# nidium/libapenetwork

Hardware: AMD Instinct MI355X
Metric: LZ4 GiB/s device-resident (compress+decompress), 1M×64KiB blocks, 1/2/4/8 GPU (higher is better)
Workload: dtype u8

## Files before the change

libapenetwork_amd/csrc/lz4_encode.hip:

```cpp
#include "lz4_gpu_internal.h"
#include <type_traits>

namespace apelz4 {

#ifdef APE_LZ4_STATS
__device__ unsigned long long g_enc_stats[16];
hipError_t enc_stats_read(unsigned long long *out, int reset) {
    hipError_t e = hipMemcpyFromSymbol(out, HIP_SYMBOL(g_enc_stats), sizeof(g_enc_stats));
    if (e == hipSuccess && reset) {
        unsigned long long z[16] = {0};
        e = hipMemcpyToSymbol(HIP_SYMBOL(g_enc_stats), z, sizeof(z));
    }
    return e;
}
#endif

namespace {

constexpr int kWavesPerEu = 7;

constexpr uint32_t kEagerLen = 12;
static_assert(kEagerLen + 4u == 16u, "in[T-4, T+kEagerLen) is one 16-byte load (loadv)");
constexpr uint32_t kEagerL = 12;
constexpr uint32_t kExt2 = 64;
constexpr uint32_t kGroups = 16;
constexpr uint32_t kRingE = 1024;
static_assert((kRingE & (kRingE - 1u)) == 0u && kRingE < 65536u,
              "the ring holds recent input, not the block's window (DESIGN.md 3.1.1)");
constexpr int kSmall = 128;
constexpr uint32_t kQ = 128;
constexpr uint32_t kFetchAt = 48, kEmitAll = 80, kChunkRecs = 64u / 4u;
static_assert((kQ & (kQ - 1u)) == 0u, "record ring indexed by & (kQ - 1)");
static_assert(kEmitAll - 1u + 2u * kChunkRecs <= kQ, "walker -> emitter record ring overflow");
static_assert(kFetchAt < kEmitAll, "a fetch precedes emit_all");
constexpr int kEmitEvery = 8;
constexpr uint32_t kStage = 512;
constexpr uint32_t kStageAlloc = kStage + 16u + 16u + 64u;


constexpr uint32_t I_TRUNC = 1u << 7, I_HASHABLE = 1u << 13;
static_assert(kEagerLen + kExt2 < 128u, "len fits 7 bits");

struct __attribute__((aligned(16))) EncLds {
    uint32_t ring[kRingE / 4 + 16];
    uint16_t tab[kHSize];
    uint2 info[64];
    uint2 q[kQ];
    uint32_t qn[2];
    uint8_t __attribute__((aligned(16))) stage[kStageAlloc];
};

template <int N>
__device__ __forceinline__ void vm_wait() {
    static_assert(N >= 0 && N < 16, "vmcnt");
    __builtin_amdgcn_s_waitcnt(N | (7 << 4) | (15 << 8));
}

__device__ __forceinline__ void shift_bytes(const uint32_t (&L)[8], int d, uint32_t (&X)[8]) {
    uint32_t T[8];
#pragma unroll
    for (int k = 0; k < 8; k++) T[k] = L[k];
    const bool down = d >= 0;
    const int ad = down ? d : -d, w = ad >> 2;
    const uint32_t r = (uint32_t)ad & 3u;
#pragma unroll
    for (int bit = 4; bit >= 1; bit >>= 1) {
        if (w & bit) {
            if (down) {
#pragma unroll
                for (int k = 0; k < 8; k++) T[k] = (k + bit < 8) ? T[k + bit] : 0u;
            } else {
#pragma unroll
                for (int k = 7; k >= 0; k--) T[k] = (k - bit >= 0) ? T[k - bit] : 0u;
            }
        }
    }
#pragma unroll
    for (int k = 0; k < 8; k++) {
        if (down) X[k] = __builtin_amdgcn_alignbyte(k + 1 < 8 ? T[k + 1] : 0u, T[k], r);
        else X[k] = r ? __builtin_amdgcn_alignbyte(T[k], k >= 1 ? T[k - 1] : 0u, 4u - r) : T[k];
    }
}

template <bool SMALL>
__device__ __forceinline__ void load32(gcu8 *in, int n, int pos, uint32_t (&X)[8],
                                       bool fast = false) {
    if (!SMALL && fast) {
        gcu8 *q = in + (uint32_t)pos;
        const uint4 a = gload16(q), b = gload16(q + 16);
        X[0] = a.x; X[1] = a.y; X[2] = a.z; X[3] = a.w;
        X[4] = b.x; X[5] = b.y; X[6] = b.z; X[7] = b.w;
        return;
    }
    if (SMALL) {
#pragma unroll
        for (int k = 0; k < 8; k++) X[k] = 0;
#pragma unroll
        for (int k = 0; k < 32; k++) {
            const int q = pos + k;
            if (q >= 0 && q < n) X[k >> 2] |= (uint32_t)in[(uint32_t)q] << (8 * (k & 3));
        }
        return;
    }
    const int ca = pos < 0 ? 0 : (pos > n - 32 ? n - 32 : pos);
    gcu8 *q = in + (uint32_t)ca;
    const uint4 a = gload16(q), b = gload16(q + 16);
    const uint32_t L[8] = {a.x, a.y, a.z, a.w, b.x, b.y, b.z, b.w};
    if (ca == pos) {
#pragma unroll
        for (int k = 0; k < 8; k++) X[k] = L[k];
    } else {
        const int d = pos - ca;
        shift_bytes(L, d < -31 ? -31 : (d > 31 ? 31 : d), X);
        if (d > 31 || d < -31) {
#pragma unroll
            for (int k = 0; k < 8; k++) X[k] = 0;
        }
    }
}

__device__ __forceinline__ uint32_t ffbl(uint32_t d) {
    uint32_t r;
    asm("v_ffbl_b32 %0, %1" : "=v"(r) : "v"(d));
    return r;
}
__device__ __forceinline__ uint32_t ffbh(uint32_t d) {
    uint32_t r;
    asm("v_ffbh_u32 %0, %1" : "=v"(r) : "v"(d));
    return r;
}

template <int K0, int NA, int NB>
__device__ __forceinline__ uint32_t first_diff_bit(const uint32_t (&A)[NA], const uint32_t (&B)[NB]) {
// ... 613 lines not shown
    E.pend = 0;
    const uint32_t s0 = E.o0 & 15u, end = s0 + E.tot;
    gu8 *out = B.dst + (E.o0 - s0);
    const uint32_t c0 = 16u * (uint32_t)lane;
    const uint64_t bigm = E.bigm;
    const uint32_t nfull = end >> 4;
    const bool head = E.part && s0 != 0u;
    if ((uint32_t)lane < umin(nfull, kStage / 16u + 1u) && !(head && lane == 0))
        gstore16(out + c0, *(const uint4 *)(S.stage + c0));
    if (head || (bigm && (end & 15u) && nfull <= kStage / 16u)) {
        const uint32_t pc = (head && lane == 0) ? 0u : 16u * nfull;
        const bool act = (head && lane == 0) || (bigm && (end & 15u) && lane == 1);
        const uint4 w = *(const uint4 *)(S.stage + (act ? pc : 0u));
        const uint32_t W[4] = {w.x, w.y, w.z, w.w};
#pragma unroll
        for (uint32_t t = 0; t < 16u; t++)
            if (act && pc + t >= s0 && pc + t < end) out[pc + t] = (uint8_t)(W[t >> 2] >> (8 * (t & 3)));
    }
    if (bigm) {
        vm_wait<0>();
        for (uint64_t m = bigm; m; m &= m - 1) {
            const int j = __builtin_ctzll(m);
            emit_one(B, lane, E.o0 - s0 + lane_val(E.r, j), lane_val(E.ba, j), lane_val(E.lit, j),
                     lane_val(E.mlm4, j), lane_val(E.off, j));
        }
        E.part = true;
    } else {
        if (lane == 0) {
            const uint4 t = *(const uint4 *)(S.stage + 16u * nfull);
            *(uint4 *)S.stage = t;
        }
        E.part = head && nfull == 0u;
    }
}

__device__ __forceinline__ void emit_step(EncLds &S, const Blk &B, int lane, Emit &E) {
    if (E.pend == 1) emit_lits(S, lane, E);
    else if (E.pend == 2) emit_heads(S, lane, E);
    else if (E.pend == 3) emit_copy(S, B, lane, E);
}
__device__ __forceinline__ void emit_all(EncLds &S, const Blk &B, int lane, Emit &E) {
    if (E.pend == 1) emit_lits(S, lane, E);
    if (E.pend == 2) emit_heads(S, lane, E);
    if (E.pend == 3) emit_copy(S, B, lane, E);
}

__device__ __forceinline__ void emit_tail(EncLds &S, const Blk &B, int lane, Emit &E) {
    const uint32_t s0 = E.o & 15u;
    if (!E.part && s0 != 0u && (uint32_t)lane < s0)
        B.dst[E.o - s0 + (uint32_t)lane] = S.stage[lane];
}

__device__ __forceinline__ void prefix_history(EncLds &S, const Blk &B, int lane) {
    const uint32_t D = 64u * (uint32_t)B.k0;
    constexpr int kU = 8;
    for (uint32_t v0 = 0; v0 < D; v0 += 192u * kU) {
        uint2 x[kU];
        bool ok[kU];
#pragma unroll
        for (int u = 0; u < kU; u++) {
            const uint32_t v = v0 + 192u * u + 3u * (uint32_t)lane;
            ok[u] = v < D && v + 8u <= B.un;
            x[u] = gload8(B.in + (ok[u] ? v : 0u));
        }
#pragma unroll
        for (int u = 0; u < kU; u++) {
            const uint32_t v = v0 + 192u * u + 3u * (uint32_t)lane;
            if (ok[u]) S.tab[hashk(x[u].x, x[u].y)] = (uint16_t)v;
        }
    }
    const uint32_t p = D - 64u + (uint32_t)lane;
    const uint8_t by = B.in[p];
    ((uint8_t *)S.ring)[p & (kRingE - 1)] = by;
    if (((D - 64u) & (kRingE - 1)) == 0u) ((uint8_t *)S.ring)[kRingE + lane] = by;
}

__device__ __forceinline__ void cdict_history(EncLds &S, const Blk &B, int lane) {
    const uint32_t p = B.D - 64u + (uint32_t)lane;
    const uint8_t by = B.win[p];
    ((uint8_t *)S.ring)[p & (kRingE - 1)] = by;
    if (((B.D - 64u) & (kRingE - 1)) == 0u) ((uint8_t *)S.ring)[kRingE + lane] = by;
}

template <bool SMALL, bool ACC, bool EXT = false>
__device__ __forceinline__ void encode_block(EncLds &S, const Blk &B, int wave, int lane,
                                             int *result, int *tail) {
    STATS_DECL
    const int k0 = B.k0;
    const int nch = B.nr >= (uint32_t)kMinLength ? B.nch : k0;
    const int nsteps = k0 + ((nch - k0 + 3) & ~1);

    if (wave == 1) {
        PSet P0, P1;
        auto pstep = [&](auto fast, int s, PSet &cur, PSet &nxt) {
            constexpr bool F = decltype(fast)::value;
            vm_wait<3>();
            STAT(9);
            prod_ring<F>(S, B, s + 2, lane, cur.X);
            uint32_t X6[6];
            prod_own(S, s + 1, lane, X6);
            prod_lookup<SMALL, F, EXT>(S, B, s + 2, lane, cur.X, cur.cT, cur.jL, cur.h, cur.Y);
            prod_load<SMALL, F, EXT>(B, s + 4, lane, cur.X);
            STAT(5);
            vm_wait<4>();
            STAT(9);
            prod_measure<SMALL, F, EXT>(S, B, s + 1, lane, X6, nxt.Y, nxt.cT, nxt.jL, nxt.h, nxt.q);
            STAT(5);
            __syncthreads();
            STAT(6);
            prod_stage2_issue<SMALL, F, EXT>(S, B, s + 1, lane, nxt.q, nxt.E);
            STAT(7);
            vm_wait<3>();
            STAT(9);
            prod_finish<SMALL, F, EXT>(S, B, s, lane, cur.q, cur.E);
            STAT(7);
            __syncthreads();
            STAT(8);
        };
        if constexpr (EXT) {
            if (k0 > 0) cdict_history(S, B, lane);
        } else {
            if (k0 > 0) prefix_history(S, B, lane);
        }
        if (nch > k0) {
            prod_load<SMALL, false, EXT>(B, k0, lane, P0.X);
            prod_load<SMALL, false, EXT>(B, k0 + 1, lane, P1.X);
            prod_ring(S, B, k0, lane, P0.X);
            prod_lookup<SMALL, false, EXT>(S, B, k0, lane, P0.X, P0.cT, P0.jL, P0.h, P0.Y);
            prod_load<SMALL, false, EXT>(B, k0 + 2, lane, P0.X);
            prod_ring(S, B, k0 + 1, lane, P1.X);
            prod_lookup<SMALL, false, EXT>(S, B, k0 + 1, lane, P1.X, P1.cT, P1.jL, P1.h, P1.Y);
            prod_load<SMALL, false, EXT>(B, k0 + 3, lane, P1.X);
            prod_ring(S, B, k0 + 2, lane, P0.X);
            uint32_t X6[6];
            prod_own(S, k0, lane, X6);
            prod_measure<SMALL, false, EXT>(S, B, k0, lane, X6, P0.Y, P0.cT, P0.jL, P0.h, P0.q);
            prod_stage2_issue<SMALL, false, EXT>(S, B, k0, lane, P0.q, P0.E);
        }
        __builtin_amdgcn_s_waitcnt(0);
        __syncthreads();
        constexpr int kFastEnd = 328;
        const int nfast_abs = SMALL ? 0 : (int)umin((uint32_t)(B.n >= kFastEnd ? (B.n - kFastEnd) / 64 + 1 : 0),
                                                    (uint32_t)nsteps);
        const int nfast = nfast_abs > k0 ? k0 + ((nfast_abs - k0) & ~1) : k0;
        int s = k0;
        for (; s < nfast; s += 2) {
            pstep(std::true_type{}, s, P0, P1);
            pstep(std::true_type{}, s + 1, P1, P0);
        }
        for (; s < nsteps; s += 2) {
            pstep(std::false_type{}, s, P0, P1);
            pstep(std::false_type{}, s + 1, P1, P0);
        }
        STATS_FLUSH_TID(g_enc_stats, 64);
        return;
    }
    if (wave == 0) {
        Walk W;
        uint32_t qn = 0;
        W.q = 64u * (uint32_t)k0;
        W.anchor = W.q;
        WalkOut O;
        __syncthreads();
        const int s2 = nch + 1;
        __syncthreads();
        __syncthreads();
        int s = k0 + 1;
        for (; s < s2; s++) {
            walk_chain<ACC, EXT>(S, B, s - 1, lane, W, O);
            STAT(0);
            __syncthreads();
            STAT(4);
            walk_finish<ACC>(B, s - 1, lane, W, O);
            walk_publish(S, B, s - 1, lane, O, qn);
            STAT_ADD(11, __popcll(O.members));
            STAT(1);
            STAT_ADD(10, 3);
            __syncthreads();
            STAT(3);
        }
        for (; s < nsteps; s++) {
            __syncthreads();
            __syncthreads();
        }
        STATS_FLUSH(g_enc_stats);
        return;
    }
    Emit E;
    E.o = 0;
    E.ein = 64u * (uint32_t)k0;
    E.qc = 0;
    E.last = k0;
    E.overflow = false;
    E.part = false;
    E.pend = 0;
    E.nv = false;
    E.o0 = E.tot = 0;
    E.bigm = 0;
    E.r = E.lit = E.mlm4 = E.off = E.ba = 0;
    __syncthreads();
    for (int s = k0; s < nsteps; s++) {
        const uint32_t qr = (uint32_t)__builtin_amdgcn_readfirstlane(S.qn[0]);
        const uint32_t avail = umax(qr, E.qc) - E.qc;
        if (E.pend == 0) {
            if (avail != 0u && (avail >= kFetchAt || s - E.last >= kEmitEvery)) {
                emit_fetch(S, B, lane, E, avail, s >= 12 ? 64u * (uint32_t)(s - 12) : 0u);
                E.last = s;
            }
        } else if (avail >= kEmitAll) {
            emit_all(S, B, lane, E);
        } else {
            emit_step(S, B, lane, E);
        }
        STAT(2);
        __syncthreads();
        STAT(14);
        if (E.pend == 1 || E.pend == 3) emit_step(S, B, lane, E);
        STAT(12);
        __syncthreads();
        STAT(15);
    }
    emit_all(S, B, lane, E);
    {
        const uint32_t rlo = B.nch > 16 ? 64u * (uint32_t)(B.nch - 16) : 0u;
        for (uint32_t left = (uint32_t)__builtin_amdgcn_readfirstlane(umax(S.qn[0], S.qn[1])) - E.qc; left;) {
            const uint32_t qc0 = E.qc;
            emit_fetch(S, B, lane, E, left, rlo);
            emit_all(S, B, lane, E);
            left -= E.qc - qc0;
        }
    }
    if (!E.overflow) emit_tail(S, B, lane, E);
    uint32_t last_run = 0;
    if (!E.overflow) {
        const uint32_t anchor = E.ein;
        const uint32_t lit = B.un - anchor;
        last_run = lit;
        const uint32_t hdr = 1u + ext_bytes(lit);
        const uint32_t total = E.o + hdr + lit;
        if (total > B.cap) {
            E.overflow = true;
        } else {
            if (lane == 0) {
                B.dst[E.o] = (uint8_t)((lit < 15u ? lit : 15u) << 4);
                put_len(B.dst + E.o + 1, lit);
            }
            wave_copy(B.in, B.dst, anchor, E.o + hdr, lit, lane);
            E.o = total;
        }
    }
    if (lane == 0) {
        *result = E.overflow ? 0 : (int)E.o;
        if (tail) *tail = E.overflow ? 0 : (int)last_run;
    }
    STAT_ADD(13, 1);
    STATS_FLUSH_TID(g_enc_stats, 128);
}

}

template <bool ACC>
__global__ void __launch_bounds__(192) __attribute__((amdgpu_waves_per_eu(kWavesPerEu)))
lz4_encode_kernel(BlockArgs a) {
    __shared__ EncLds S;
    const int b = blockIdx.x;
    const int tid = threadIdx.x;
    const int lane = tid & 63, wave = __builtin_amdgcn_readfirstlane(tid >> 6);

    Blk B;
    B.in = (gcu8 *)(a.src ? a.src[b] : a.src_base + (size_t)b * a.src_stride);
    B.dst = (gu8 *)(a.dst ? a.dst[b] : a.dst_base + (size_t)b * a.dst_stride);
    const int nr = a.src_size[b];
    const int icap = a.dst_cap ? a.dst_cap[b] : (int)a.dst_stride;
    if (nr < 0 || nr > kMaxBlock || icap < 0) {
        if (tid == 0) a.result[b] = (nr > kMaxBlock) ? kErange : 0;
        return;
    }
    int D = 0;
    if (a.dict_size) {
        const int pre = a.dict_size[b];
        D = (pre > 0 ? (pre < kMaxBlock - nr ? pre : kMaxBlock - nr) : 0) & ~63;
        if (D < 64) D = 0;
    }
    B.in -= D;
    B.n = D + nr;
    B.nr = (uint32_t)nr;
    B.k0 = D / 64;
    B.stride = ACC ? (a.accel < (1 << 20) ? (uint32_t)a.accel : 1u << 20) : 1u;
    B.cap = (uint32_t)icap;
    B.un = (uint32_t)B.n;
    B.mstart = B.un >= 12 ? B.un - 12 : 0;
    B.mlimit = B.un >= 5 ? B.un - 5 : 0;
    B.nch = (B.n + 63) / 64;

    for (int i = tid; i < kHSize / 8; i += 192) ((uint4 *)S.tab)[i] = make_uint4(0, 0, 0, 0);
    for (int i = tid; i < (int)(kRingE / 16 + 4); i += 192) ((uint4 *)S.ring)[i] = make_uint4(0, 0, 0, 0);
    if (tid == 0) S.qn[0] = S.qn[1] = 0u;
    __syncthreads();
    int *const tail = a.tail ? a.tail + b : nullptr;
    if (B.n < kSmall) encode_block<true, ACC>(S, B, wave, lane, &a.result[b], tail);
    else encode_block<false, ACC>(S, B, wave, lane, &a.result[b], tail);
}

__global__ void __launch_bounds__(192) __attribute__((amdgpu_waves_per_eu(kWavesPerEu)))
lz4_encode_cdict_kernel(BlockArgs a, const uint8_t *cd) {
    __shared__ EncLds S;
    const int b = blockIdx.x;
    const int tid = threadIdx.x;
    const int lane = tid & 63, wave = __builtin_amdgcn_readfirstlane(tid >> 6);

    const CDictHdr H = *(const CDictHdr *)cd;
#include "lz4_encode_cdict.inc"
}

__global__ void __launch_bounds__(192) __attribute__((amdgpu_waves_per_eu(kWavesPerEu)))
lz4_encode_cdicts_kernel(BlockArgs a, const uint8_t *const *cdicts) {
    __shared__ EncLds S;
    const int b = blockIdx.x;
    const int tid = threadIdx.x;
    const int lane = tid & 63, wave = __builtin_amdgcn_readfirstlane(tid >> 6);

    gcu8 *cd = (gcu8 *)message_object(cdicts, b);
    if (!cd) {
        if (tid == 0) a.result[b] = 0;
        return;
    }
    const CDictHdr H = object_header<true>(cd);
#include "lz4_encode_cdict.inc"
}

hipError_t launch_encode_cdicts(const BlockArgs &a, const void *const *cdicts, hipStream_t s) {
    if (a.nblocks <= 0) return hipSuccess;
    hipLaunchKernelGGL(lz4_encode_cdicts_kernel, dim3(a.nblocks), dim3(192), 0, s, a,
                       (const uint8_t *const *)cdicts);
    return hipGetLastError();
}

hipError_t launch_encode_cdict(const BlockArgs &a, const void *cdict, hipStream_t s) {
    if (a.nblocks <= 0) return hipSuccess;
    hipLaunchKernelGGL(lz4_encode_cdict_kernel, dim3(a.nblocks), dim3(192), 0, s, a,
                       (const uint8_t *)cdict);
    return hipGetLastError();
}

hipError_t launch_encode(const BlockArgs &a, hipStream_t s) {
    if (a.nblocks <= 0) return hipSuccess;
    if (a.accel > 1)
        hipLaunchKernelGGL(lz4_encode_kernel<true>, dim3(a.nblocks), dim3(192), 0, s, a);
    else
        hipLaunchKernelGGL(lz4_encode_kernel<false>, dim3(a.nblocks), dim3(192), 0, s, a);
    return hipGetLastError();
}

}
```

libapenetwork_amd/csrc/lz4_encode_cdict.inc:

```
    if (H.magic != kCdMagic || H.D > kCdMaxWin || (H.D & 63u) != 0u || H.max_src < 1u ||
        H.max_src > (uint32_t)kMaxBlock || H.D + H.max_src > (uint32_t)kMaxBlock) {
        if (tid == 0) a.result[b] = 0;
        return;
    }
    const int nr = a.src_size[b];
    const int icap = a.dst_cap[b];
    if (nr < 0 || nr > (int)H.max_src || icap < 0) {
        if (tid == 0) a.result[b] = (nr > (int)H.max_src) ? kErange : 0;
        return;
    }
    const int D = (int)H.D;
    Blk B;
    B.win = (gcu8 *)(cd + kCdWin + kCdFront);
    B.D = (uint32_t)D;
    B.in = (gcu8 *)a.src[b] - D;
    B.dst = (gu8 *)a.dst[b];
    B.n = D + nr;
    B.nr = (uint32_t)nr;
    B.k0 = D / 64;
    B.stride = 1u;
    B.cap = (uint32_t)icap;
    B.un = (uint32_t)B.n;
    B.mstart = B.un >= 12 ? B.un - 12 : 0;
    B.mlimit = B.un >= 5 ? B.un - 5 : 0;
    B.nch = (B.n + 63) / 64;

    const uint4 *img = (const uint4 *)(cd + kCdTab);
    for (int i = tid; i < kHSize / 8; i += 192) ((uint4 *)S.tab)[i] = img[i];
    for (int i = tid; i < (int)(kRingE / 16 + 4); i += 192) ((uint4 *)S.ring)[i] = make_uint4(0, 0, 0, 0);
    if (tid == 0) S.qn[0] = S.qn[1] = 0u;
    __syncthreads();
    if (B.n < kSmall) encode_block<true, false, true>(S, B, wave, lane, &a.result[b], nullptr);
    else encode_block<false, false, true>(S, B, wave, lane, &a.result[b], nullptr);
```

libapenetwork_amd/csrc/lz4_gpu_internal.h:

```cpp
#pragma once
#include <hip/hip_runtime.h>
#include <stdint.h>

namespace apelz4 {

constexpr int kMinMatch = 4;
constexpr int kLastLiterals = 5;
constexpr int kMFLimit = 12;
constexpr int kMinLength = 13;
constexpr int kMaxBlock = 65536;
constexpr int kErange = -2147483647 - 1;

typedef __attribute__((address_space(1))) const uint8_t gcu8;
typedef __attribute__((address_space(1))) uint8_t gu8;
typedef uint32_t u32x4_u __attribute__((ext_vector_type(4), aligned(1)));
typedef uint32_t u32x2_u __attribute__((ext_vector_type(2), aligned(1)));
typedef uint32_t u32_u __attribute__((aligned(1)));

__device__ __forceinline__ uint4 gload16(gcu8 *p) {
    const u32x4_u v = *(__attribute__((address_space(1))) const u32x4_u *)p;
    return make_uint4(v.x, v.y, v.z, v.w);
}
__device__ __forceinline__ uint2 gload8(gcu8 *p) {
    const u32x2_u v = *(__attribute__((address_space(1))) const u32x2_u *)p;
// ... 3 lines not shown
    return *(__attribute__((address_space(1))) const u32_u *)p;
}
__device__ __forceinline__ void gstore16(gu8 *p, uint4 v) {
    u32x4_u w;
    w.x = v.x; w.y = v.y; w.z = v.z; w.w = v.w;
    *(__attribute__((address_space(1))) u32x4_u *)p = w;
}
__device__ __forceinline__ void gstore4(gu8 *p, uint32_t v) {
    *(__attribute__((address_space(1))) u32_u *)p = v;
}

__device__ __forceinline__ int lane_id() { return (int)__lane_id(); }

__device__ __forceinline__ uint64_t wave_ballot(bool c) { return __builtin_amdgcn_ballot_w64(c); }
__device__ __forceinline__ bool wave_any(bool c) { return __builtin_amdgcn_ballot_w64(c) != 0; }
__device__ __forceinline__ bool lane_in(uint64_t m) { return __builtin_amdgcn_inverse_ballot_w64(m); }

template <int CTRL, int ROW_MASK = 0xF>
__device__ __forceinline__ uint32_t dpp(uint32_t old, uint32_t v) {
    return (uint32_t)__builtin_amdgcn_update_dpp((int)old, (int)v, CTRL, ROW_MASK, 0xF, false);
}
template <int CTRL>
__device__ __forceinline__ uint32_t dpp_z(uint32_t v) {
    return (uint32_t)__builtin_amdgcn_mov_dpp((int)v, CTRL, 0xF, 0xF, true);
}
constexpr int kDppRowShr1 = 0x111, kDppRowShr2 = 0x112, kDppRowShr4 = 0x114,
              kDppRowShr8 = 0x118, kDppBcast15 = 0x142, kDppBcast31 = 0x143,
              kDppWaveShr1 = 0x138, kDppWaveShl1 = 0x130;

__device__ __forceinline__ uint32_t wave_incl_sum(uint32_t x) {
    x += dpp<kDppRowShr1>(0u, x);
    x += dpp<kDppRowShr2>(0u, x);
    x += dpp<kDppRowShr4>(0u, x);
    x += dpp<kDppRowShr8>(0u, x);
    x += dpp<kDppBcast15, 0xA>(0u, x);
    x += dpp<kDppBcast31, 0xC>(0u, x);
    return x;
}

__device__ __forceinline__ uint32_t umax(uint32_t a, uint32_t b) { return a > b ? a : b; }
__device__ __forceinline__ uint32_t umin(uint32_t a, uint32_t b) { return a < b ? a : b; }

__device__ __forceinline__ uint32_t wave_incl_max(uint32_t x) {
    x = umax(x, dpp<kDppRowShr1>(0u, x));
    x = umax(x, dpp<kDppRowShr2>(0u, x));
    x = umax(x, dpp<kDppRowShr4>(0u, x));
    x = umax(x, dpp<kDppRowShr8>(0u, x));
    x = umax(x, dpp<kDppBcast15, 0xA>(0u, x));
    x = umax(x, dpp<kDppBcast31, 0xC>(0u, x));
    return x;
}

__device__ __forceinline__ uint32_t wave_shr1(uint32_t x, uint32_t first) {
    return dpp<kDppWaveShr1>(first, x);
}

__device__ __forceinline__ uint32_t wave_excl_scan(uint32_t v) {
    return wave_shr1(wave_incl_sum(v), 0u);
}

__device__ __forceinline__ uint32_t lane_val(uint32_t v, int l) {
    return (uint32_t)__builtin_amdgcn_readlane((int)v, l);
}

__device__ __forceinline__ uint32_t wave_first(uint32_t v) {
    return (uint32_t)__builtin_amdgcn_readfirstlane((int)v);
}
template <class T>
__device__ __forceinline__ T *wave_uniform(T *p) {
    const uint64_t v = (uint64_t)p;
    return (T *)((uint64_t)wave_first((uint32_t)(v >> 32)) << 32 | wave_first((uint32_t)v));
}

constexpr int kHSize = 7328;
static_assert(kHSize < 8192 && kHSize % 8 == 0, "table size");
constexpr int kKey = 7;

__device__ __forceinline__ uint32_t hashk(uint32_t x0, uint32_t x1) {
    static_assert(kKey == 7, "hashk covers bytes 0..6");
    const uint32_t hi = __builtin_amdgcn_alignbyte(x1, x0, 3u);
    const uint32_t v = (uint32_t)__umul24(x0, 0x9E3779u) + (uint32_t)__umul24(hi, 0xC2B2AEu) +
                       (uint32_t)__umul24((x1 >> 16) & 0xFFu, 0x27D4EBu);
    return __umulhi(v, (uint32_t)kHSize);
}

constexpr uint32_t kCdMagic = 0x44435A4Cu;
constexpr uint32_t kCdTab = 16u, kCdWin = kCdTab + 2u * (uint32_t)kHSize;
constexpr uint32_t kCdFront = 16u, kCdBack = 256u;
constexpr uint32_t kCdMaxWin = (uint32_t)kMaxBlock - 64u;
constexpr uint32_t kCdSize = kCdWin + kCdFront + (uint32_t)kMaxBlock + kCdBack;
static_assert(kCdWin % 16u == 0u && kCdSize % 16u == 0u, "prepared dictionary regions");
struct CDictHdr {
    uint32_t magic, D, max_src, zero;
};
__device__ __forceinline__ const uint8_t *message_object(const uint8_t *const *objs, int b) {
    const uint8_t *cd = wave_uniform(objs[b]);
    return ((uint64_t)cd & 15u) ? nullptr : cd;
}
template <bool PER, class P>
__device__ __forceinline__ CDictHdr object_header(P *cd) {
    if constexpr (!PER) {
        return *(const CDictHdr *)cd;
    } else {
        const uint4 v = gload16((gcu8 *)cd);
        return CDictHdr{wave_first(v.x), wave_first(v.y), wave_first(v.z), wave_first(v.w)};
    }
}
__host__ __device__ inline int cdict_window(int dict_size, int max_src) {
    const int room = kMaxBlock - max_src;
    return (dict_size < room ? dict_size : room) & ~63;
}

#ifdef APE_LZ4_STATS
#define STATS_DECL uint64_t st_t_ = clock64(); uint64_t st_acc_[16] = {0};
#define STAT(i) do { uint64_t t_ = clock64(); st_acc_[i] += t_ - st_t_; st_t_ = t_; } while (0)
#define STAT_ADD(i, v) (st_acc_[i] += (uint64_t)(v))
#define STATS_FLUSH(arr) STATS_FLUSH_TID(arr, 0)
#define STATS_FLUSH_TID(arr, t) do { if (threadIdx.x == (t)) { _Pragma("unroll") for (int i_ = 0; i_ < 16; i_++) if (st_acc_[i_]) atomicAdd(&(arr)[i_], (unsigned long long)st_acc_[i_]); } } while (0)
#else
#define STATS_DECL
#define STAT(i) do {} while (0)
#define STAT_ADD(i, v) do {} while (0)
#define STATS_FLUSH(arr) do {} while (0)
#define STATS_FLUSH_TID(arr, t) do {} while (0)
#endif
hipError_t stats_read(int which, unsigned long long *out, int reset);

struct BlockArgs {
    const char *const *src;
    char *const *dst;
    const char *src_base;
    char *dst_base;
    size_t src_stride, dst_stride;
    const int *src_size;
    const int *dst_cap;
    const int *target;
    const long long *frame_off;
    const char *const *dict;
    const int *dict_size;
    int fast;
    int accel;
    int *result;
    int nblocks;
    int *tail;
};

hipError_t launch_decode(const BlockArgs &a, bool partial, hipStream_t s);
hipError_t launch_decode_chain(const BlockArgs &a, int nconn, int nq, hipStream_t s);
hipError_t launch_encode(const BlockArgs &a, hipStream_t s);
hipError_t launch_encode_cdict(const BlockArgs &a, const void *cdict, hipStream_t s);
hipError_t launch_encode_cdicts(const BlockArgs &a, const void *const *cdicts, hipStream_t s);
hipError_t launch_cdict_prepare(const char *dict, int dict_size, int max_src, void *cdict,
                                hipStream_t s);
hipError_t launch_cdict_prepare_batch(const char *const *dict, const int *dict_size, int max_src,
                                      void *cdicts, size_t stride, int n, hipStream_t s);
hipError_t launch_encode_exact(const BlockArgs &a, hipStream_t s);
constexpr int kHcCap = 272;
constexpr int kHcHashBits = 14;
constexpr int kHcMaxDepth = 256, kHcDefaultDepth = 64;
constexpr int kHcTable = 1 << kHcHashBits;
__device__ __forceinline__ uint32_t hc_hash(uint32_t x) {
    return (x * 2654435761u) >> (32 - kHcHashBits);
}
__device__ __forceinline__ uint32_t len_bytes(uint32_t v) { return v >= 15u ? (v - 15u) / 255u + 1u : 0u; }
__device__ __forceinline__ uint32_t first_diff(uint32_t x) { return (uint32_t)__builtin_ctz(x) >> 3; }
constexpr size_t kHcChainBytes = (size_t)kMaxBlock * sizeof(uint16_t);
constexpr size_t kHcSlotBytes = kHcChainBytes + (size_t)kMaxBlock * sizeof(uint32_t);
struct HcArgs {
    const char *const *src;
    const int *src_size;
    char *const *dst;
    const int *dst_cap;
    int *result;
    int nblocks, depth;
    uint16_t *chain;
    uint32_t *match;
    const int *prefix;
    int *tail;
};
hipError_t launch_encode_hc(const HcArgs &a, hipStream_t s, hipEvent_t *ev = nullptr);
constexpr size_t kHcOptSlotBytes = kHcSlotBytes + (size_t)kMaxBlock * sizeof(uint32_t);
struct HcOptArgs {
    HcArgs a;
    uint32_t *cost;
};
hipError_t launch_encode_hc_opt(const HcOptArgs &o, hipStream_t s, hipEvent_t *ev = nullptr);

constexpr uint32_t kHdMagic = 0x44485A4Cu;
constexpr uint32_t kHdHead = 16u, kHdChain = kHdHead + 2u * (1u << kHcHashBits);
constexpr uint32_t kHdWin = kHdChain + 2u * (uint32_t)kMaxBlock;
constexpr uint32_t kHdSize = kHdWin + kCdFront + (uint32_t)kMaxBlock + kCdBack;
static_assert(kHdChain % 16u == 0u && kHdWin % 16u == 0u && kHdSize % 16u == 0u,
              "prepared high-ratio dictionary regions");
__host__ __device__ inline int hc_cdict_window(int dict_size, int max_src) {
    const int room = kMaxBlock - max_src;
    return dict_size < room ? dict_size : room;
}
inline size_t hc_cdict_chain_entries(int max_src) { return ((size_t)max_src + 3 + 7) & ~(size_t)7; }
inline size_t hc_cdict_match_entries(int max_src) { return ((size_t)max_src + 3) & ~(size_t)3; }
inline size_t hc_cdict_slot_bytes(int max_src) {
    return hc_cdict_chain_entries(max_src) * sizeof(uint16_t) +
           hc_cdict_match_entries(max_src) * sizeof(uint32_t);
}
constexpr int kHcdThreads = 256;
inline int hc_cdict_groups(int max_src) { return (max_src + kHcdThreads - 1) / kHcdThreads; }
struct HcDictArgs {
    const char *const *src;
    const int *src_size;
    char *const *dst;
    const int *dst_cap;
    int *result;
    int nblocks, depth;
    int max_src;
    const uint8_t *cdict;
    uint16_t *chain;
    uint32_t *match;
    uint32_t chain_stride, match_stride;
};
hipError_t launch_hc_cdict_prepare(const char *dict, int dict_size, int max_src, void *cdict,
                                   hipStream_t s);
hipError_t launch_hc_cdict_prepare_batch(const char *const *dict, const int *dict_size,
                                         int max_src, void *cdicts, size_t stride, int n,
                                         hipStream_t s);
hipError_t launch_encode_hc_cdict(const HcDictArgs &a, hipStream_t s,
                                  const uint8_t *const *cdicts = nullptr);
inline size_t hc_cdict_cost_entries(int max_src) { return ((size_t)max_src + 3) & ~(size_t)3; }
inline size_t hc_cdict_opt_slot_bytes(int max_src) {
    return hc_cdict_slot_bytes(max_src) + hc_cdict_cost_entries(max_src) * sizeof(uint32_t);
}
struct HcDictOptArgs {
    HcDictArgs a;
    uint32_t *cost;
// ... 123 lines not shown
```

libapenetwork_amd/csrc/lz4_runtime.hip:

```cpp
#include <initializer_list>
#include <mutex>
#include <stdarg.h>
#include <stdio.h>
#include <string.h>
#include <vector>

#include "../../include/ape_lz4_gpu.h"
#include "lz4_gpu_internal.h"
#include "lz4_gpu_shim.h"

using namespace apelz4;

namespace {

thread_local char g_err[256] = "";

void set_err(const char *what, hipError_t e) {
    snprintf(g_err, sizeof g_err, "%s: %s", what, e == hipSuccess ? "ok" : hipGetErrorString(e));
}

__attribute__((format(printf, 1, 2))) int einval(const char *fmt, ...) {
    va_list ap;
    va_start(ap, fmt);
    vsnprintf(g_err, sizeof g_err, fmt, ap);
// ... 1104 lines not shown
    if (int rc = ready_strided("compress_batch_strided_dev", a)) return rc;
    return finish_launch(launch_encode(a, (hipStream_t)stream), "lz4_encode_kernel");
}

int APE_LZ4_decompress_safe_batch_strided_dev(const char *d_src, size_t src_stride,
                                              const int *d_compressedSize, char *d_dst,
                                              size_t dst_stride, const int *d_maxDecompressedSize,
                                              int *d_result, int nblocks, void *stream) {
    BlockArgs a = strided_args(d_src, src_stride, d_compressedSize, d_dst, dst_stride,
                               d_maxDecompressedSize, d_result, nblocks);
    if (int rc = ready_strided("decompress_safe_batch_strided_dev", a)) return rc;
    return finish_launch(launch_decode(a, false, (hipStream_t)stream), "lz4_decode_kernel");
}

size_t APE_LZ4_frame_scratch_size(int nblocks) {
    return nblocks < 0 ? 0 : (size_t)frame_scratch_elems(nblocks) * sizeof(long long);
}

int APE_LZ4_frame_offsets_dev(const int *d_compressedSize, long long *d_off,
                              void *d_scratch, int nblocks, void *stream) {
    if (nblocks < 0 || !d_compressedSize || !d_off || !d_scratch)
        return einval("frame_offsets_dev: invalid argument (a null array or a negative count, "
                      "nblocks %d)", nblocks);
    if (int rc = check_device()) return rc;
    return finish_launch(launch_frame_offsets(d_compressedSize, d_off, (long long *)d_scratch,
                                              nblocks, (hipStream_t)stream),
                         "frame offsets");
}

int APE_LZ4_frame_pack_strided_dev(const char *d_comp, size_t comp_stride,
                                   const int *d_compressedSize, const long long *d_off,
                                   char *d_frames, int nblocks, void *stream) {
    if (int rc = check_arrays("frame_pack_strided_dev", nblocks,
                              {d_comp, d_compressedSize, d_off, d_frames}))
        return rc;
    if (int rc = check_device()) return rc;
    return finish_launch(launch_frame_pack(d_comp, comp_stride, d_compressedSize, d_off,
                                           d_frames, nblocks, (hipStream_t)stream),
                         "frame pack");
}

int APE_LZ4_decompress_safe_frames_dev(const char *d_frames, const long long *d_off,
                                       char *d_dst, size_t dst_stride,
                                       const int *d_maxDecompressedSize, int *d_result,
                                       int nblocks, void *stream) {
    BlockArgs a = strided_args(d_frames, 0, nullptr, d_dst, dst_stride, d_maxDecompressedSize,
                               d_result, nblocks);
    a.frame_off = d_off;
    if (int rc = ready_strided("decompress_safe_frames_dev", a)) return rc;
    return finish_launch(launch_decode(a, false, (hipStream_t)stream), "lz4_decode_kernel");
}

int APE_LZ4_compress_batch_host(const char *const *h_src, const int *h_srcSize,
                                char *const *h_dst, const int *h_dstCap, int *h_result,
                                int nblocks) {
    return host_batch("compress_batch_host", 0, 1, h_src, h_srcSize, h_dst, h_dstCap, nullptr,
                      h_result, nblocks);
}

int APE_LZ4_decompress_safe_batch_host(const char *const *h_src, const int *h_compressedSize,
                                       char *const *h_dst, const int *h_maxDecompressedSize,
                                       int *h_result, int nblocks) {
    return host_batch("decompress_safe_batch_host", 1, 1, h_src, h_compressedSize, h_dst,
                      h_maxDecompressedSize, nullptr, h_result, nblocks);
}

int APE_LZ4_synth_blocks_dev(char *d_out, size_t stride, int blockSize, long long first_block,
                             int nblocks, int kind, void *stream) {
    if (nblocks < 0 || blockSize < 0 || blockSize > kMaxBlock || (nblocks > 0 && !d_out) ||
        stride < (size_t)blockSize)
        return einval("synth_blocks_dev: nblocks %d of %d bytes (0..%d) at %p with stride %zu",
                      nblocks, blockSize, kMaxBlock, d_out, stride);
    if (int rc = check_device()) return rc;
    return finish_launch(launch_synth(d_out, stride, blockSize, first_block, nblocks, kind,
                                      (hipStream_t)stream),
                         "lz4_synth_kernel");
}

#ifdef APE_LZ4_STATS
}
namespace apelz4 {
hipError_t dec_stats_read(unsigned long long *out, int reset);
hipError_t enc_stats_read(unsigned long long *out, int reset);
}
extern "C" {
int APE_LZ4_debug_stats(int which, unsigned long long *out16, int reset) {
    hipError_t e = which ? apelz4::enc_stats_read(out16, reset) : apelz4::dec_stats_read(out16, reset);
    return e == hipSuccess ? 0 : -1;
}
#endif

int ape_lz4_gpu_compress_one(const char *src, char *dst, int n, int cap, int accel, int *rt) {
    int res = 0;
    *rt = host_batch("compress_one", 0, accel, &src, &n, &dst, &cap, nullptr, &res, 1);
    return res;
}

int ape_lz4_gpu_decompress_one(const char *src, char *dst, int csize, int cap, int partial,
                               int target, int *rt) {
    int res = 0;
    *rt = host_batch("decompress_one", partial ? 2 : 1, 1, &src, &csize, &dst, &cap,
                     partial ? &target : nullptr, &res, 1);
    return res;
}

}
```

Before: 148.0.

## Assign encoder wave roles dynamically by per-SIMD load across CUs

Each encode workgroup reads its hardware CU and SIMD IDs and consults a global per-SIMD load table. It then permutes the walker, producer and emitter roles so the heavy producer wave lands on the least-loaded SIMD, and releases the load weight when it finishes. This targets imbalance when several resident blocks put their producer waves on the same SIMD. In exchange it adds global atomics per block, an extra barrier, and getreg reads, and it only runs for blocks of at least 32 KiB in auto mode.

```diff
diff --git a/libapenetwork_amd/csrc/lz4_encode.hip b/libapenetwork_amd/csrc/lz4_encode.hip
--- a/libapenetwork_amd/csrc/lz4_encode.hip
+++ b/libapenetwork_amd/csrc/lz4_encode.hip
@@ -10,6 +10,40 @@
     if (e == hipSuccess && reset) {
         unsigned long long z[16] = {0};
         e = hipMemcpyToSymbol(HIP_SYMBOL(g_enc_stats), z, sizeof(z));
+    }
+    return e;
+}
+#endif
+
+__device__ int g_enc_load[kEncCus * 4];
+static int g_role_mode = kEncRoleAuto;
+int enc_role_mode_set(int mode) {
+    if (mode < 0 || mode > kEncNPerms) return -1;
+    const int old = g_role_mode;
+    g_role_mode = mode;
+    return old;
+}
+hipError_t enc_loads_read(int *out) {
+    return hipMemcpyFromSymbol(out, HIP_SYMBOL(g_enc_load), sizeof(g_enc_load));
+}
+#ifdef APE_LZ4_STATS
+__device__ unsigned long long g_enc_place[64];
+__device__ int g_enc_prod[kEncCus * 4];
+__device__ int g_enc_seen[kEncCus];
+hipError_t enc_place_read(unsigned long long *out, int reset) {
+    unsigned long long h[64];
+    static int seen[kEncCus];
+    hipError_t e = hipMemcpyFromSymbol(h, HIP_SYMBOL(g_enc_place), sizeof(h));
+    if (e == hipSuccess) e = hipMemcpyFromSymbol(seen, HIP_SYMBOL(g_enc_seen), sizeof(seen));
+    if (e != hipSuccess) return e;
+    h[53] = 0;
+    for (int i = 0; i < kEncCus; i++) h[53] += seen[i] != 0;
+    for (int i = 0; i < 64; i++) out[i] = h[i];
+    if (reset) {
+        for (int i = 0; i < 64; i++) h[i] = 0;
+        for (int i = 0; i < kEncCus; i++) seen[i] = 0;
+        e = hipMemcpyToSymbol(HIP_SYMBOL(g_enc_place), h, sizeof(h));
+        if (e == hipSuccess) e = hipMemcpyToSymbol(HIP_SYMBOL(g_enc_seen), seen, sizeof(seen));
     }
     return e;
 }
@@ -47,8 +81,12 @@
     uint2 info[64];
     uint2 q[kQ];
     uint32_t qn[2];
+    uint8_t simd[4];
+    uint32_t perm;
     uint8_t __attribute__((aligned(16))) stage[kStageAlloc];
 };
+
+static_assert(sizeof(EncLds) <= 35 * 512, "35 LDS granules of 512 bytes: 9 blocks per CU");
 
 template <int N>
 __device__ __forceinline__ void vm_wait() {
@@ -828,15 +866,83 @@
     if (((B.D - 64u) & (kRingE - 1)) == 0u) ((uint8_t *)S.ring)[kRingE + lane] = by;
 }
 
+__device__ __forceinline__ uint32_t hw_simd() {
+    return __builtin_amdgcn_s_getreg(4 | 4 << 6 | (2 - 1) << 11);
+}
+__device__ __forceinline__ uint32_t hw_cu() {
+    const uint32_t cu = __builtin_amdgcn_s_getreg(4 | 8 << 6 | (8 - 1) << 11);
+    const uint32_t xcc = __builtin_amdgcn_s_getreg(20 | 0 << 6 | (4 - 1) << 11);
+    return (xcc << 8 | cu) & (uint32_t)(kEncCus - 1);
+}
+
+[[maybe_unused]] constexpr int kEncPlaceMin = 32768;
+__device__ __forceinline__ bool place_wanted(int mode, int nr) {
+#ifdef APE_LZ4_STATS
+    return true;
+#else
+    return mode == kEncRoleAuto && nr >= kEncPlaceMin;
+#endif
+}
+__device__ __forceinline__ int fixed_role(int mode, int wave) {
+    return enc_role(mode == kEncRoleAuto ? 0 : (int)umin((uint32_t)mode - 1u, kEncNPerms - 1u), wave);
+}
+
+__device__ __forceinline__ int place_begin(EncLds &S, int tid, int wave) {
+    if ((tid & 63) == 0) S.simd[wave] = (uint8_t)hw_simd();
+    int ld = 0;
+    if (tid < 4) ld = __hip_atomic_load(&g_enc_load[hw_cu() * 4u + (uint32_t)tid], __ATOMIC_RELAXED,
+                                        __HIP_MEMORY_SCOPE_AGENT);
+    return ld;
+}
+__device__ __forceinline__ int place_roles(EncLds &S, int mode, int ld, int tid, int wave) {
+    if (wave == 0) {
+        const int load[4] = {(int)lane_val((uint32_t)ld, 0), (int)lane_val((uint32_t)ld, 1),
+                             (int)lane_val((uint32_t)ld, 2), (int)lane_val((uint32_t)ld, 3)};
+        if (tid == 0) {
+            const int sd[3] = {S.simd[0] & 3, S.simd[1] & 3, S.simd[2] & 3};
+            const int k = mode != kEncRoleAuto ? mode - 1 : enc_place_roles(sd, load);
+            const uint32_t cu = hw_cu();
+#pragma unroll
+            for (int w = 0; w < kEncRoles; w++)
+                atomicAdd(&g_enc_load[cu * 4u + (uint32_t)sd[w]], enc_weight(enc_role(k, w)));
+            uint32_t post = (uint32_t)k | cu << 16;
+#ifdef APE_LZ4_STATS
+            {
+                int pw = 0;
+                for (int w = 0; w < kEncRoles; w++) if (enc_role(k, w) == 1) pw = w;
+                const int c = atomicAdd(&g_enc_prod[cu * 4u + (uint32_t)sd[pw]], 1);
+                post |= (uint32_t)(c < 0 ? 0 : c > 15 ? 15 : c) << 8;
+                g_enc_seen[cu] = 1;
+                if (sd[0] == sd[1] || sd[0] == sd[2] || sd[1] == sd[2]) atomicAdd(&g_enc_place[48], 1ull);
+                atomicAdd(&g_enc_place[49], 1ull);
+                atomicMax(&g_enc_place[50], (unsigned long long)umax(umax(S.simd[0], S.simd[1]), S.simd[2]));
+                atomicMax(&g_enc_place[51], (unsigned long long)__builtin_amdgcn_s_getreg(20 | (4 - 1) << 11));
+                atomicOr(&g_enc_place[52], (unsigned long long)__builtin_amdgcn_s_getreg(4 | 8 << 6 | (8 - 1) << 11));
+            }
+#endif
+            S.perm = post;
+        }
+    }
+    __syncthreads();
+    const int k = (int)umin(wave_first(S.perm) & 7u, (uint32_t)kEncNPerms - 1u);
+    return enc_role(k, wave);
+}
+__device__ __forceinline__ uint32_t place_entry(const EncLds &S, int wave) {
+    return (wave_first(S.perm) >> 16 & (uint32_t)(kEncCus - 1)) * 4u + (wave_first(S.simd[wave]) & 3u);
+}
+__device__ __forceinline__ void place_release(const EncLds &S, int wave, int role, int lane) {
+    if (lane == 0) atomicSub(&g_enc_load[place_entry(S, wave)], enc_weight(role));
+}
+
 template <bool SMALL, bool ACC, bool EXT = false>
-__device__ __forceinline__ void encode_block(EncLds &S, const Blk &B, int wave, int lane,
+__device__ __forceinline__ void encode_block(EncLds &S, const Blk &B, int role, int lane,
                                              int *result, int *tail) {
     STATS_DECL
     const int k0 = B.k0;
     const int nch = B.nr >= (uint32_t)kMinLength ? B.nch : k0;
     const int nsteps = k0 + ((nch - k0 + 3) & ~1);
 
-    if (wave == 1) {
+    if (role == 1) {
         PSet P0, P1;
         auto pstep = [&](auto fast, int s, PSet &cur, PSet &nxt) {
             constexpr bool F = decltype(fast)::value;
@@ -890,6 +996,9 @@
                                                     (uint32_t)nsteps);
         const int nfast = nfast_abs > k0 ? k0 + ((nfast_abs - k0) & ~1) : k0;
         int s = k0;
+#ifdef APE_LZ4_STATS
+        const uint64_t place_t0 = clock64();
+#endif
         for (; s < nfast; s += 2) {
             pstep(std::true_type{}, s, P0, P1);
             pstep(std::true_type{}, s + 1, P1, P0);
@@ -898,10 +1007,19 @@
             pstep(std::false_type{}, s, P0, P1);
             pstep(std::false_type{}, s + 1, P1, P0);
         }
-        STATS_FLUSH_TID(g_enc_stats, 64);
+#ifdef APE_LZ4_STATS
+        if (lane == 0 && nsteps > k0) {
+            const uint32_t c = wave_first(S.perm) >> 8 & 15u;
+            atomicAdd(&g_enc_place[c], 1ull);
+            atomicAdd(&g_enc_place[16 + c], (unsigned long long)(clock64() - place_t0));
+            atomicAdd(&g_enc_place[32 + c], (unsigned long long)(nsteps - k0));
+        }
+        if (lane == 0) atomicSub(&g_enc_prod[place_entry(S, (int)(threadIdx.x >> 6))], 1);
+#endif
+        STATS_FLUSH_TID(g_enc_stats, threadIdx.x & ~63u);
         return;
     }
-    if (wave == 0) {
+    if (role == 0) {
         Walk W;
         uint32_t qn = 0;
         W.q = 64u * (uint32_t)k0;
@@ -929,7 +1047,7 @@
             __syncthreads();
             __syncthreads();
         }
-        STATS_FLUSH(g_enc_stats);
+        STATS_FLUSH_TID(g_enc_stats, threadIdx.x & ~63u);
         return;
     }
     Emit E;
@@ -1000,7 +1118,7 @@
         if (tail) *tail = E.overflow ? 0 : (int)last_run;
     }
     STAT_ADD(13, 1);
-    STATS_FLUSH_TID(g_enc_stats, 128);
+    STATS_FLUSH_TID(g_enc_stats, threadIdx.x & ~63u);
 }
 
 }
@@ -1039,13 +1157,17 @@
     B.mlimit = B.un >= 5 ? B.un - 5 : 0;
     B.nch = (B.n + 63) / 64;
 
+    const bool placed = place_wanted(a.role_mode, nr);
+    const int ld = placed ? place_begin(S, tid, wave) : 0;
     for (int i = tid; i < kHSize / 8; i += 192) ((uint4 *)S.tab)[i] = make_uint4(0, 0, 0, 0);
     for (int i = tid; i < (int)(kRingE / 16 + 4); i += 192) ((uint4 *)S.ring)[i] = make_uint4(0, 0, 0, 0);
     if (tid == 0) S.qn[0] = S.qn[1] = 0u;
     __syncthreads();
+    const int role = placed ? place_roles(S, a.role_mode, ld, tid, wave) : fixed_role(a.role_mode, wave);
     int *const tail = a.tail ? a.tail + b : nullptr;
-    if (B.n < kSmall) encode_block<true, ACC>(S, B, wave, lane, &a.result[b], tail);
-    else encode_block<false, ACC>(S, B, wave, lane, &a.result[b], tail);
+    if (B.n < kSmall) encode_block<true, ACC>(S, B, role, lane, &a.result[b], tail);
+    else encode_block<false, ACC>(S, B, role, lane, &a.result[b], tail);
+    if (placed) place_release(S, wave, role, lane);
 }
 
 __global__ void __launch_bounds__(192) __attribute__((amdgpu_waves_per_eu(kWavesPerEu)))
@@ -1075,22 +1197,31 @@
 #include "lz4_encode_cdict.inc"
 }
 
-hipError_t launch_encode_cdicts(const BlockArgs &a, const void *const *cdicts, hipStream_t s) {
-    if (a.nblocks <= 0) return hipSuccess;
+static BlockArgs with_role_mode(const BlockArgs &a) {
+    BlockArgs b = a;
+    b.role_mode = g_role_mode;
+    return b;
+}
+
+hipError_t launch_encode_cdicts(const BlockArgs &a0, const void *const *cdicts, hipStream_t s) {
+    if (a0.nblocks <= 0) return hipSuccess;
+    const BlockArgs a = with_role_mode(a0);
     hipLaunchKernelGGL(lz4_encode_cdicts_kernel, dim3(a.nblocks), dim3(192), 0, s, a,
                        (const uint8_t *const *)cdicts);
     return hipGetLastError();
 }
 
-hipError_t launch_encode_cdict(const BlockArgs &a, const void *cdict, hipStream_t s) {
-    if (a.nblocks <= 0) return hipSuccess;
+hipError_t launch_encode_cdict(const BlockArgs &a0, const void *cdict, hipStream_t s) {
+    if (a0.nblocks <= 0) return hipSuccess;
+    const BlockArgs a = with_role_mode(a0);
     hipLaunchKernelGGL(lz4_encode_cdict_kernel, dim3(a.nblocks), dim3(192), 0, s, a,
                        (const uint8_t *)cdict);
     return hipGetLastError();
 }
 
-hipError_t launch_encode(const BlockArgs &a, hipStream_t s) {
-    if (a.nblocks <= 0) return hipSuccess;
+hipError_t launch_encode(const BlockArgs &a0, hipStream_t s) {
+    if (a0.nblocks <= 0) return hipSuccess;
+    const BlockArgs a = with_role_mode(a0);
     if (a.accel > 1)
         hipLaunchKernelGGL(lz4_encode_kernel<true>, dim3(a.nblocks), dim3(192), 0, s, a);
     else
diff --git a/libapenetwork_amd/csrc/lz4_encode_cdict.inc b/libapenetwork_amd/csrc/lz4_encode_cdict.inc
--- a/libapenetwork_amd/csrc/lz4_encode_cdict.inc
+++ b/libapenetwork_amd/csrc/lz4_encode_cdict.inc
@@ -25,10 +25,14 @@
     B.mlimit = B.un >= 5 ? B.un - 5 : 0;
     B.nch = (B.n + 63) / 64;
 
+    const bool placed = place_wanted(a.role_mode, nr);
+    const int ld = placed ? place_begin(S, tid, wave) : 0;
     const uint4 *img = (const uint4 *)(cd + kCdTab);
     for (int i = tid; i < kHSize / 8; i += 192) ((uint4 *)S.tab)[i] = img[i];
     for (int i = tid; i < (int)(kRingE / 16 + 4); i += 192) ((uint4 *)S.ring)[i] = make_uint4(0, 0, 0, 0);
     if (tid == 0) S.qn[0] = S.qn[1] = 0u;
     __syncthreads();
-    if (B.n < kSmall) encode_block<true, false, true>(S, B, wave, lane, &a.result[b], nullptr);
-    else encode_block<false, false, true>(S, B, wave, lane, &a.result[b], nullptr);
+    const int role = placed ? place_roles(S, a.role_mode, ld, tid, wave) : fixed_role(a.role_mode, wave);
+    if (B.n < kSmall) encode_block<true, false, true>(S, B, role, lane, &a.result[b], nullptr);
+    else encode_block<false, false, true>(S, B, role, lane, &a.result[b], nullptr);
+    if (placed) place_release(S, wave, role, lane);
diff --git a/libapenetwork_amd/csrc/lz4_gpu_internal.h b/libapenetwork_amd/csrc/lz4_gpu_internal.h
--- a/libapenetwork_amd/csrc/lz4_gpu_internal.h
+++ b/libapenetwork_amd/csrc/lz4_gpu_internal.h
@@ -109,6 +109,48 @@
     const uint32_t v = (uint32_t)__umul24(x0, 0x9E3779u) + (uint32_t)__umul24(hi, 0xC2B2AEu) +
                        (uint32_t)__umul24((x1 >> 16) & 0xFFu, 0x27D4EBu);
     return __umulhi(v, (uint32_t)kHSize);
+}
+
+constexpr int kEncRoles = 3, kEncNPerms = 6;
+constexpr uint8_t kEncPerms[kEncNPerms][kEncRoles] = {{0, 1, 2}, {0, 2, 1}, {1, 0, 2},
+                                                      {1, 2, 0}, {2, 0, 1}, {2, 1, 0}};
+constexpr int kEncWeightWalker = 32, kEncWeightProducer = 98, kEncWeightEmitter = 13;
+__host__ __device__ inline int enc_weight(int role) {
+    return role == 0 ? kEncWeightWalker : role == 1 ? kEncWeightProducer : kEncWeightEmitter;
+}
+constexpr int kEncCus = 2048;
+constexpr int kEncRoleAuto = 0;
+constexpr uint64_t enc_perm_roles() {
+    uint64_t v = 0;
+    for (int k = 0; k < kEncNPerms; k++)
+        for (int w = 0; w < kEncRoles; w++) v |= (uint64_t)kEncPerms[k][w] << (6 * k + 2 * w);
+    return v;
+}
+constexpr uint64_t enc_perm_index() {
+    uint64_t v = 0;
+    for (int k = 0; k < kEncNPerms; k++) {
+        int p = 0, w = 0;
+        for (int i = 0; i < kEncRoles; i++) {
+            if (kEncPerms[k][i] == 1) p = i;
+            if (kEncPerms[k][i] == 0) w = i;
+        }
+        v |= (uint64_t)k << (4 * (3 * p + w));
+    }
+    return v;
+}
+__host__ __device__ inline int enc_role(int k, int wave) {
+    constexpr uint64_t roles = enc_perm_roles();
+    return (int)(roles >> (6 * k + 2 * wave) & 3u);
+}
+__host__ __device__ inline int enc_place_roles(const int (&simd)[kEncRoles], const int (&load)[4]) {
+    const int ld[3] = {load[simd[0] & 3], load[simd[1] & 3], load[simd[2] & 3]};
+    int p = 1;
+    if (ld[0] < ld[p]) p = 0;
+    if (ld[2] < ld[p]) p = 2;
+    const int a = p == 0 ? 1 : 0, b = p == 2 ? 1 : 2;
+    const int w = ld[b] < ld[a] ? b : a;
+    constexpr uint64_t index = enc_perm_index();
+    return (int)(index >> (4 * (3 * p + w)) & 7u);
 }
 
 constexpr uint32_t kCdMagic = 0x44435A4Cu;
@@ -170,11 +212,14 @@
     int *result;
     int nblocks;
     int *tail;
+    int role_mode;
 };
 
 hipError_t launch_decode(const BlockArgs &a, bool partial, hipStream_t s);
 hipError_t launch_decode_chain(const BlockArgs &a, int nconn, int nq, hipStream_t s);
 hipError_t launch_encode(const BlockArgs &a, hipStream_t s);
+int enc_role_mode_set(int mode);
+hipError_t enc_loads_read(int *out);
 hipError_t launch_encode_cdict(const BlockArgs &a, const void *cdict, hipStream_t s);
 hipError_t launch_encode_cdicts(const BlockArgs &a, const void *const *cdicts, hipStream_t s);
 hipError_t launch_cdict_prepare(const char *dict, int dict_size, int max_src, void *cdict,
diff --git a/libapenetwork_amd/csrc/lz4_runtime.hip b/libapenetwork_amd/csrc/lz4_runtime.hip
--- a/libapenetwork_amd/csrc/lz4_runtime.hip
+++ b/libapenetwork_amd/csrc/lz4_runtime.hip
@@ -1210,13 +1210,24 @@
 namespace apelz4 {
 hipError_t dec_stats_read(unsigned long long *out, int reset);
 hipError_t enc_stats_read(unsigned long long *out, int reset);
+hipError_t enc_place_read(unsigned long long *out, int reset);
 }
 extern "C" {
+int ape_lz4_enc_place_stats(unsigned long long *out64, int reset) {
+    return apelz4::enc_place_read(out64, reset) == hipSuccess ? 0 : -1;
+}
 int APE_LZ4_debug_stats(int which, unsigned long long *out16, int reset) {
     hipError_t e = which ? apelz4::enc_stats_read(out16, reset) : apelz4::dec_stats_read(out16, reset);
     return e == hipSuccess ? 0 : -1;
 }
 #endif
+
+int ape_lz4_enc_role_mode(int mode) { return enc_role_mode_set(mode); }
+int ape_lz4_enc_role_loads(int *out, int n) {
+    if (!out || n < kEncCus * 4) return -1;
+    if (check_device()) return -1;
+    return enc_loads_read(out) == hipSuccess ? 0 : -1;
+}
 
 int ape_lz4_gpu_compress_one(const char *src, char *dst, int n, int cap, int accel, int *rt) {
     int res = 0;
```

Result: no change. 149.4 (median of 6 runs) (+1.0%).
